# ag14774/OpenCL-Lattice-Boltzmann

Measured on AMD Instinct MI355X. Metric: MLUPS, higher is better.
Workload: dtype f32

## Files before the change

opencl-lattice-boltzmann_amd/csrc/core_interval.h:

```cpp
#pragma once

#if defined(__HIPCC__) || defined(__CUDACC__)
#define LBM_CORE_HD __host__ __device__ inline
#else
#define LBM_CORE_HD inline
#endif

namespace lbm {

struct CoreInterval {
  int kc0, kc1;
};

LBM_CORE_HD CoreInterval core_interval(int ys, int ye, int L, int ny, bool up, bool twinned, int accel_row, int accel_row_b,
                                       bool accel_next) {
  const int n = ye - ys, d = up ? 1 : -1;
  const int lead = twinned ? 0 : L - 1, sf = twinned ? 1 : 2;
  const int r0 = up ? ys - lead : ye - 1 + lead;
  const CoreInterval none = {0, 0};
  if (n <= 0 || L < 2) return none;
  int lo = lead + L - 1, hi = n + lead - 1;
  const int k_steady = sf * (L - 1) + 1;
  if (lo < k_steady) lo = k_steady;
  if (up) {
// ... 3 lines not shown
    if (lo < kmin) lo = kmin;
  } else {
    const int kmax = (r0 - 1) - 1;
    if (hi > kmax) hi = kmax;
    const int kmin = r0 - (ny - 2) - 1;
    if (lo < kmin) lo = kmin;
  }
  if (hi - lo + 1 < 2) return none;
  const int Lacc = accel_next ? L : L - 1;
  int c0[2], c1[2], nc = 0;
  const int arows[2] = {accel_row, accel_row_b};
  for (int i = 0; i < 2; i++) {
    const int A = arows[i];
    if (A < 0 || A >= ny || Lacc <= 0) continue;
    const int kA = (A - r0) * d;
    if (kA + Lacc - 1 < lo || kA > hi) continue;
    int j = nc++;
    if (j == 1 && kA < c0[0]) { c0[1] = c0[0]; c1[1] = c1[0]; j = 0; }
    c0[j] = kA;
    c1[j] = kA + Lacc - 1;
  }
  int best0 = 0, best1 = 0;
  int start = lo;
  for (int i = 0; i <= nc; i++) {
    const int end = i < nc ? c0[i] : hi + 1;
    if (end - start > best1 - best0) { best0 = start; best1 = end; }
    if (i < nc && c1[i] + 1 > start) start = c1[i] + 1;
  }
  if (best1 - best0 < 2) return none;
  const CoreInterval r = {best0, best1};
  return r;
}

}
```

opencl-lattice-boltzmann_amd/csrc/d2q9_kernels.h:

```cpp
#pragma once
#include <type_traits>

#include <hip/hip_runtime.h>
#include <stdint.h>

#include "core_interval.h"

namespace lbm {

constexpr int kBlock = 256;

struct StepArgs {
  const float *src;
  float *dst;
  const uint8_t *mask;
  const float *south_src[3];
  const float *north_src[3];
  float *partials;
  unsigned long long plane_stride;
  unsigned long long row_stride;
  int nx, rows;
  int y_begin, y_count;
  int y_split, y_begin2;
  int accel_row;
// ... 397 lines not shown
    }
  }
}

struct Step2Args {
  const float *src;
  float *dst;
  const uint8_t *mask;
  float *partials1;
  float *partials2;
  unsigned long long plane_stride, row_stride;
  int nx, ny;
  int strips, lanes_out;
  const int *chunk_start;
  int nchunks;
  int nbands, units_per_band;
  int skip_chunk;
  int accel_row;
  int accel_row_b;
  int accel_next;
  float omega, aw1, aw2;
  const int *edge_chunk_start;
  int edge_nchunks, edge_units, edge_skip;
  int edge_partial_off;
  const struct HaloPeer *peer;
  uint32_t seq, wait_seq;
  int peer_mode, peer_buf;
  const unsigned long long *clean_bits;
  int clean_words;
  const int *vmap;
  const int *vtab;
  int strips_edge;
  int core_loop;
};

struct UnitSel {
  const int *chunk_start;
  int bid, nbands, units_per_band, skip, partial_off;
  bool edge;
};
template <bool PUSH>
__device__ __forceinline__ UnitSel select_unit(const Step2Args &a, int edge_wgs) {
  UnitSel u{a.chunk_start, (int)blockIdx.x, a.nbands, a.units_per_band, a.skip_chunk, 0, false};
  if constexpr (PUSH) {
    if (u.bid < edge_wgs) {
      u.edge = true;
      u.chunk_start = a.edge_chunk_start;
      u.nbands = 1;
      u.units_per_band = edge_wgs;
      u.skip = a.edge_skip;
      u.partial_off = a.edge_partial_off;
    } else {
      u.bid -= edge_wgs;
    }
  }
  return u;
}

__device__ __forceinline__ void push_chunk(const Step2Args *la, int ys, int ye, int xcol, bool owner) {
  drain_stores();
  const HaloPeer *pp = uniform_ptr(la->peer);
  const int hi0 = __builtin_amdgcn_readfirstlane(pp->row_hi0);
  const int lo0 = __builtin_amdgcn_readfirstlane(pp->row_lo0);
  const int rows = __builtin_amdgcn_readfirstlane(pp->push_rows);
  const int buf = __builtin_amdgcn_readfirstlane(la->peer_buf) & 1;
  const int side = ys >= hi0 ? 1 : 0;
// ... 944 lines not shown
  float h0, h1, h2;
  uint32_t m;
};
template <bool NTL, bool HALO = true>
__device__ __forceinline__ void issue_pair_loads(const Step2Args &a, int r, int xcol, int xhalo_w, int xhalo_e, int lane, PairLoads &in) {
  const size_t ps = a.plane_stride, rs = a.row_stride;
  const int r_s = (r == 0) ? a.ny - 1 : r - 1;
  const int r_n = (r == a.ny - 1) ? 0 : r + 1;
  const float *Rc = a.src + (size_t)r * rs, *Rs = a.src + (size_t)r_s * rs, *Rn = a.src + (size_t)r_n * rs;
  unsigned xb = (unsigned)xcol * 4u;
  asm volatile("" : "+v"(xb));
  auto ld = [&](const float *p) {
    if (NTL) return __builtin_nontemporal_load(reinterpret_cast<const v2f *>(at_byte(p, xb)));
    return *reinterpret_cast<const v2f *>(at_byte(p, xb));
  };
  in.c[0] = ld(Rc); in.c[1] = ld(Rc + ps); in.c[3] = ld(Rc + 3 * ps);
  in.c[2] = ld(Rs + 2 * ps); in.c[5] = ld(Rs + 5 * ps); in.c[6] = ld(Rs + 6 * ps);
  in.c[4] = ld(Rn + 4 * ps); in.c[7] = ld(Rn + 7 * ps); in.c[8] = ld(Rn + 8 * ps);
  {
    unsigned mb = (unsigned)(xcol & ~3);
    asm volatile("" : "+v"(mb));
    in.m = *reinterpret_cast<const uint32_t *>(a.mask + (size_t)r * a.nx + mb);
  }
  in.h0 = in.h1 = in.h2 = 0.f;
  if (HALO && (lane == 0 || lane == 63)) {
    const bool lo = (lane == 0);
    in.h0 = lo ? Rc[1 * ps + xhalo_w] : Rc[3 * ps + xhalo_e];
    in.h1 = lo ? Rs[5 * ps + xhalo_w] : Rs[6 * ps + xhalo_e];
    in.h2 = lo ? Rn[8 * ps + xhalo_w] : Rn[7 * ps + xhalo_e];
  }
}

typedef __attribute__((address_space(1))) v2f global_v2f;
constexpr int kPairSlotFloats = 128;
constexpr int kPairWinFloats = 9 * kPairSlotFloats;
struct PairWindow { v2f mid[3], S0[3], S1[3]; };
struct __attribute__((packed, aligned(4))) f2u { float x, y; };
__device__ __forceinline__ v2f lds_pair(const float *p) { return *reinterpret_cast<const v2f *>(p); }
__device__ __forceinline__ v2f lds_pair_shifted(const float *p) {
  const f2u t = *reinterpret_cast<const f2u *>(p);
  v2f r = {t.x, t.y};
  return r;
}
__device__ __forceinline__ void lds_pair_put(float *p, v2f v) { *reinterpret_cast<v2f *>(p) = v; }

__device__ __forceinline__ void issue_pair_loads_at(const float *Rc, size_t ps, size_t rs, int xcol, PairLoads &in) {
  unsigned xb = (unsigned)xcol * 4u;
  asm volatile("" : "+v"(xb));
  auto ld = [&](const float *p) {
    unsigned long long pk = (unsigned long long)p;
    asm volatile("" : "+s"(pk));
    return *(const global_v2f *)(pk + xb);
  };
  const float *const Rs = Rc - rs, *const Rn = Rc + rs;
  in.c[0] = ld(Rc); in.c[1] = ld(Rc + ps); in.c[3] = ld(Rc + 3 * ps);
  in.c[2] = ld(Rs + 2 * ps); in.c[5] = ld(Rs + 5 * ps); in.c[6] = ld(Rs + 6 * ps);
  in.c[4] = ld(Rn + 4 * ps); in.c[7] = ld(Rn + 7 * ps); in.c[8] = ld(Rn + 8 * ps);
}

constexpr int deep_halo_lanes(int D) { return D / 2; }
constexpr bool deep_edge_loads(int D) { return 2 * deep_halo_lanes(D) < D; }
constexpr int deep_lds_windows(int D) { return D - 1 < 4 ? D - 1 : 4; }

__device__ __forceinline__ bool strip_rows_clean(const unsigned long long *bits, int words, int strip, int lo, int hi, int ny) {
  if (bits == nullptr || hi - lo >= ny) return false;
  const unsigned long long *w = bits + (size_t)strip * words;
  unsigned long long any = 0;
  auto range = [&](int r0, int r1) {
    for (int i = r0 >> 6; i <= (r1 - 1) >> 6; i++) {
      const int b0 = r0 - 64 * i > 0 ? r0 - 64 * i : 0, b1 = r1 - 64 * i < 64 ? r1 - 64 * i : 64;
      const unsigned long long upto = b1 == 64 ? ~0ull : ((1ull << b1) - 1ull);
      any |= w[i] & upto & ~((1ull << b0) - 1ull);
    }
  };
  int l0 = lo % ny;
  if (l0 < 0) l0 += ny;
  const int l1 = l0 + (hi - lo);
// ... 21 lines not shown
    const int r = word * 64 + b;
    if (r >= rows) break;
    const uint32_t m = *reinterpret_cast<const uint32_t *>(mask + (size_t)r * nx + (xcol & ~3)) >> ((xcol & 2) * 8);
    if (__builtin_amdgcn_ballot_w64((m & 0xffffu) != 0) != 0ull) out |= 1ull << b;
  }
  if (lane == 0) bits[(size_t)strip * words + word] = out;
}

template <int D, int WL, bool UP, bool NT, bool OBST_PATHS, bool TWIN = false, int LT = 0, bool FREE = false>
__device__ __forceinline__ void deep_sweep(const Step2Args &a, const int L_arg, float *lds, float *partials, int pstride, int ys, int ye,
                                           int xcol, int xhalo_w, int xhalo_e, int lane, bool owner, int unit,
                                           const bool twinned_in = false, float *lds_twin = nullptr) {
  static_assert(LT >= 0 && LT <= D, "steady depth");
  const int L = LT > 0 ? LT : L_arg;
  const bool twinned = TWIN && twinned_in;
  const size_t ps = a.plane_stride;
  auto wrap = [&](int r) { return r < 0 ? r + a.ny : (r >= a.ny ? r - a.ny : r); };
  const int n = ye - ys, d = UP ? 1 : -1;
  const int lead = twinned ? 0 : L - 1;
  const int sf = twinned ? 1 : 2;
  const int r0 = UP ? ys - lead : ye - 1 + lead;
  const int last = n + lead + (L - 1) - 1;
  float sum[D];
  constexpr int NR = (D - 1 - WL) > 0 ? (D - 1 - WL) : 1;
  PairWindow w[NR];
  uint32_t m_mid[D - 1];
#pragma unroll
  for (int l = 0; l < D; l++) sum[l] = 0.f;
#pragma unroll
  for (int l = 0; l < D - 1; l++) m_mid[l] = 0;
#pragma unroll
  for (int l = 0; l < NR; l++) {
#pragma unroll
    for (int i = 0; i < 3; i++) w[l].mid[i] = w[l].S0[i] = w[l].S1[i] = splat2(0.f);
  }
  float *const lw = lds + 2 + 2 * lane;
  uint32_t accbits = 0, ownbits = 0;
  const uint32_t accmask = a.accel_next ? 0xffffffffu : ~(1u << (L - 1));
  const uint32_t mask_shift = (xcol & 2) * 8;
  PairLoads in;
  issue_pair_loads<false, deep_edge_loads(D)>(a, wrap(r0), xcol, xhalo_w, xhalo_e, lane, in);
  float *const mailbox = lw + WL * kPairWinFloats;
  auto window_read = [&](int l, int par, int k, v2f (&q)[6]) __attribute__((always_inline)) {
    if ((l - 1) < WL) {
      const float *W = lw + (l - 1) * kPairWinFloats;
      const float *Wp = W + (3 + 3 * par) * kPairSlotFloats;
      q[0] = lds_pair(W); q[1] = lds_pair_shifted(W + kPairSlotFloats - 1); q[2] = lds_pair_shifted(W + 2 * kPairSlotFloats + 1);
      q[3] = lds_pair(Wp); q[4] = lds_pair_shifted(Wp + kPairSlotFloats - 1); q[5] = lds_pair_shifted(Wp + 2 * kPairSlotFloats + 1);
    } else {
      const PairWindow &R = w[(l - 1) < WL ? 0 : (l - 1 - WL)];
      q[0] = R.mid[0]; q[1] = pair_from_west(R.mid[1]); q[2] = pair_from_east(R.mid[2]);
      q[3] = R.S0[0]; q[4] = pair_from_west(R.S0[1]); q[5] = pair_from_east(R.S0[2]);
      if (TWIN && twinned && k == l) {
        q[3] = lds_pair(mailbox);
        q[4] = lds_pair_shifted(mailbox + kPairSlotFloats - 1);
        q[5] = lds_pair_shifted(mailbox + 2 * kPairSlotFloats + 1);
      }
    }
  };
  v2f out[9];
#pragma unroll
  for (int kk = 0; kk < 9; kk++) out[kk] = splat2(0.f);
  auto store_row_at = [&](float *const row) __attribute__((always_inline)) {
    if (owner) {
      unsigned xb = (unsigned)xcol * 4u;
      asm volatile("" : "+v"(xb));
#pragma unroll
      for (int kk = 0; kk < 9; kk++) {
        unsigned long long pk = (unsigned long long)(row + kk * ps);
        asm volatile("" : "+s"(pk));
        global_v2f *const q = (global_v2f *)(pk + xb);
        if (NT) __builtin_nontemporal_store(out[kk], q);
        else *q = out[kk];
      }
    }
  };
  auto store_row = [&](int kprev) __attribute__((always_inline)) { store_row_at(a.dst + (size_t)(r0 + (kprev - (L - 1)) * d) * a.row_stride); };
  constexpr bool HAS_CORE = LT > 0 && FREE && !deep_edge_loads(D);
  const float *core_src = a.src;
  float *core_dst = a.dst;
  const long long core_step = UP ? (long long)a.row_stride : -(long long)a.row_stride;
  auto iteration = [&](const int k, auto lt_tag, auto core_tag) __attribute__((always_inline)) {
    constexpr int LS = decltype(lt_tag)::value;
    constexpr bool STEADY = LS > 0;
    constexpr bool CORE = decltype(core_tag)::value;
    static_assert(!CORE || (STEADY && HAS_CORE), "the CORE form is a steady form of the free sweeps");
    const int LL = STEADY ? LS : L;
    const int par = k & 1;
    v2f top[9], pre[2][6];
    uint32_t m_top;
    if (!CORE) {
      const int row0 = wrap(r0 + k * d);
      accbits = ((accbits << 1) | ((row0 == a.accel_row || row0 == a.accel_row_b) ? 1u : 0u)) & accmask;
      ownbits = (ownbits << 1) | ((k >= lead && k <= n + lead - 1) ? 1u : 0u);
    }
    if (STEADY || k >= sf) window_read(1, par, STEADY ? -1 : k, pre[1]);
    {
      v2f g[9];
      g[0] = in.c[0]; g[2] = in.c[2]; g[4] = in.c[4];
      if (deep_edge_loads(D)) {
        g[1] = pair_from_west(in.c[1], in.h0); g[5] = pair_from_west(in.c[5], in.h1); g[8] = pair_from_west(in.c[8], in.h2);
        g[3] = pair_from_east(in.c[3], in.h0); g[6] = pair_from_east(in.c[6], in.h1); g[7] = pair_from_east(in.c[7], in.h2);
      } else {
        g[1] = pair_from_west(in.c[1]); g[5] = pair_from_west(in.c[5]); g[8] = pair_from_west(in.c[8]);
        g[3] = pair_from_east(in.c[3]); g[6] = pair_from_east(in.c[6]); g[7] = pair_from_east(in.c[7]);
      }
      m_top = FREE ? 0u : in.m >> mask_shift;
      v2f t;
      if (FREE || (OBST_PATHS && __builtin_amdgcn_ballot_w64((m_top & 0xffffu) != 0) == 0ull)) t = collide2<false>(g, m_top, a.omega, !CORE && (accbits & 1u) != 0, a.aw1, a.aw2, top);
      else t = collide2<true>(g, m_top, a.omega, (accbits & 1u) != 0, a.aw1, a.aw2, top);
      if ((CORE || (ownbits & 1u)) && owner) sum[0] += t.x + t.y;
      if (CORE) {
        store_row_at(core_dst);
        issue_pair_loads_at(core_src, ps, a.row_stride, xcol, in);
        core_dst += core_step;
        core_src += core_step;
      } else {
        if (STEADY || k - 1 >= sf * (LL - 1)) store_row(k - 1);
        issue_pair_loads<false, deep_edge_loads(D)>(a, wrap(r0 + (k < last ? k + 1 : k) * d), xcol, xhalo_w, xhalo_e, lane, in);
      }
    }
#pragma unroll
    for (int l = 1; l < D; l++) {
      if (STEADY && l >= LS) break;
      if (STEADY) __builtin_amdgcn_sched_barrier(0);
      const bool final = (l == D - 1) || (l == LL - 1);
      if (!STEADY && TWIN && (l - 1) >= WL && twinned && k == l) __syncthreads();
      v2f nxt[9];
      uint32_t m_nxt = 0;
      const bool active = STEADY || k >= sf * l;
      const bool in_lds = (l - 1) < WL;
      float *const W = lw + (l - 1) * kPairWinFloats;
      float *const Wp = W + (3 + 3 * par) * kPairSlotFloats;
      PairWindow &R = w[in_lds ? 0 : (l - 1 - WL)];
      if (active) {
        const v2f (&q)[6] = pre[l & 1];
        if (l + 1 < D && !final && (STEADY || k >= sf * (l + 1))) window_read(l + 1, par, STEADY ? -1 : k, pre[(l + 1) & 1]);
        v2f g[9];
        g[0] = q[0]; g[1] = q[1]; g[3] = q[2];
        if (UP) {
          g[2] = q[3]; g[5] = q[4]; g[6] = q[5];
          g[4] = top[4]; g[8] = pair_from_west(top[8]); g[7] = pair_from_east(top[7]);
        } else {
          g[4] = q[3]; g[8] = q[4]; g[7] = q[5];
          g[2] = top[2]; g[5] = pair_from_west(top[5]); g[6] = pair_from_east(top[6]);
        }
        m_nxt = FREE ? 0u : m_mid[l - 1];
        const bool acc = !CORE && ((accbits >> l) & 1u) != 0;
        v2f t;
        if (FREE || (OBST_PATHS && __builtin_amdgcn_ballot_w64((m_nxt & 0xffffu) != 0) == 0ull)) t = collide2<false>(g, m_nxt, a.omega, acc, a.aw1, a.aw2, nxt);
        else t = collide2<true>(g, m_nxt, a.omega, acc, a.aw1, a.aw2, nxt);
        if (!final) {
          if ((CORE || ((ownbits >> l) & 1u)) && owner) sum[l] += t.x + t.y;
        } else {
          if (owner) sum[l] += t.x + t.y;
#pragma unroll
          for (int kk = 0; kk < 9; kk++) out[kk] = nxt[kk];
        }
      }
      if (in_lds) {
        lds_pair_put(W, top[0]); lds_pair_put(W + kPairSlotFloats, top[1]); lds_pair_put(W + 2 * kPairSlotFloats, top[3]);
        lds_pair_put(Wp, UP ? top[2] : top[4]);
        lds_pair_put(Wp + kPairSlotFloats, UP ? top[5] : top[8]);
        lds_pair_put(Wp + 2 * kPairSlotFloats, UP ? top[6] : top[7]);
      } else {
        R.mid[0] = top[0]; R.mid[1] = top[1]; R.mid[2] = top[3];
#pragma unroll
        for (int i = 0; i < 3; i++) R.S0[i] = R.S1[i];
        R.S1[0] = UP ? top[2] : top[4]; R.S1[1] = UP ? top[5] : top[8]; R.S1[2] = UP ? top[6] : top[7];
      }
      if (!FREE) m_mid[l - 1] = m_top;
      if (!STEADY && TWIN && twinned && k == l - 1) {
        float *const Wt = lds_twin + 2 + 2 * lane + (in_lds ? (l - 1) * kPairWinFloats + (3 + 3 * (l & 1)) * kPairSlotFloats : WL * kPairWinFloats);
        lds_pair_put(Wt, UP ? top[4] : top[2]);
        lds_pair_put(Wt + kPairSlotFloats, UP ? top[8] : top[5]);
        lds_pair_put(Wt + 2 * kPairSlotFloats, UP ? top[7] : top[6]);
      }
      if (!active || final) break;
      if (l < D - 1) {
#pragma unroll
        for (int kk = 0; kk < 9; kk++) top[kk] = nxt[kk];
        m_top = m_nxt;
      }
    }
    if (!STEADY && TWIN && twinned && k <= L - 2) __syncthreads();
  };
  const int k_steady = sf * (L - 1) + 1;
  int k = 0;
  if (LT > 0) {
    for (; k < k_steady && k <= last; k++) iteration(k, std::integral_constant<int, 0>{}, std::false_type{});
    if constexpr (HAS_CORE) {
      CoreInterval ci = {0, 0};
      if (a.core_loop) ci = core_interval(ys, ye, L, a.ny, UP, twinned, a.accel_row, a.accel_row_b, a.accel_next != 0);
      const int kc0 = __builtin_amdgcn_readfirstlane(ci.kc0), kc1 = __builtin_amdgcn_readfirstlane(ci.kc1);
      bool core_ahead = kc1 > kc0;
      for (;;) {
        const int stop = core_ahead ? kc0 : last + 1;
        for (; k < stop; k++) iteration(k, std::integral_constant<int, LT>{}, std::false_type{});
        if (!core_ahead) break;
        core_ahead = false;
        core_src = a.src + (long long)(r0 + (kc0 + 1) * d) * (long long)a.row_stride;
        core_dst = a.dst + (long long)(r0 + (kc0 - L) * d) * (long long)a.row_stride;
        for (; k < kc1; k++) iteration(k, std::integral_constant<int, LT>{}, std::true_type{});
        ownbits = (1u << L) - 1u;
        accbits = 0;
      }
    } else {
      for (; k <= last; k++) iteration(k, std::integral_constant<int, LT>{}, std::false_type{});
    }
  } else {
    for (; k <= last; k++) iteration(k, std::integral_constant<int, 0>{}, std::false_type{});
  }
  store_row(last);
#pragma unroll
  for (int l = 0; l < D; l++) {
    if (l >= L) break;
    const float s = wave_sum(sum[l]);
    if (lane == 0) partials[(size_t)l * pstride + unit] = s;
  }
}

__device__ __forceinline__ void push_chunk_pairs(const Step2Args *la, int ys, int ye, int xcol, bool owner) {
  drain_stores();
  const HaloPeer *pp = uniform_ptr(la->peer);
  const int hi0 = __builtin_amdgcn_readfirstlane(pp->row_hi0);
  const int lo0 = __builtin_amdgcn_readfirstlane(pp->row_lo0);
  const int rows = __builtin_amdgcn_readfirstlane(pp->push_rows);
  const int buf = __builtin_amdgcn_readfirstlane(la->peer_buf) & 1;
  const int side = ys >= hi0 ? 1 : 0;
  const int base = side ? hi0 : lo0;
  if (ys < base || ye > base + rows) {
    if ((threadIdx.x & 63) == 0) atomicOr(pp->wait_err, 2u);
    return;
  }
  const size_t rs = la->row_stride, ps = la->plane_stride;
  const float *own = la->dst + xcol;
  float *peer = pp->push[side][buf] + xcol;
  if (owner) {
    for (int y = ys; y < ye; y++) {
      const float *src = own + (size_t)y * rs;
      float *dst = peer + (size_t)(y - base) * rs;
      v2f v[9];
#pragma unroll
      for (int k = 0; k < 9; k++) v[k] = *reinterpret_cast<const v2f *>(src + k * ps);
// ... 54 lines not shown
  if (qw < 0) qw += q2;
  const int xcol = qw * 2;
  const int xhalo_w = (xcol == 0) ? a.nx - 1 : xcol - 1;
  const int xhalo_e = (xcol + 2 >= a.nx) ? 0 : xcol + 2;
  const bool up = __builtin_amdgcn_readfirstlane((int)((chunk & 1) == 0)) != 0;
  bool clean = false;
  if constexpr (LT > 0 && OBST_PATHS) {
    int lo, hi;
    deep_sweep_rows(up, false, LT, ys, ye, &lo, &hi);
    clean = strip_rows_clean(a.clean_bits, a.clean_words, strip, lo, hi, a.ny);
  }
  if (clean) {
    if constexpr (LT > 0 && OBST_PATHS) {
      if (up) deep_sweep<D, WL, true, NT, OBST_PATHS, false, LT, true>(a, nlev, lds, partials, pstride, ys, ye, xcol, xhalo_w, xhalo_e, lane, owner, unit);
      else deep_sweep<D, WL, false, NT, OBST_PATHS, false, LT, true>(a, nlev, lds, partials, pstride, ys, ye, xcol, xhalo_w, xhalo_e, lane, owner, unit);
    }
  } else if (up) {
    deep_sweep<D, WL, true, NT, OBST_PATHS, false, LT>(a, nlev, lds, partials, pstride, ys, ye, xcol, xhalo_w, xhalo_e, lane, owner, unit);
  } else {
    deep_sweep<D, WL, false, NT, OBST_PATHS, false, LT>(a, nlev, lds, partials, pstride, ys, ye, xcol, xhalo_w, xhalo_e, lane, owner, unit);
  }
  if constexpr (PUSH) {
    const Step2Args *la = late_args<Step2Args>();
    if (do_push) {
      push_chunk_pairs(la, ys, ye, xcol, owner);
      publish_wave_when_last(la->peer, (unsigned)la->edge_units, la->seq);
    }
  }
}

template <int D, bool NT, bool OBST_PATHS = false, int LT = 0, bool PUSH = false>
__global__ __launch_bounds__(128, 2) void d2q9_deep_twin(const Step2Args a, float *partials, int pstride, int nlev) {
  constexpr int WL = deep_lds_windows(D), HL = deep_halo_lanes(D);
  constexpr int kWaveFloats = WL * kPairWinFloats + (D - 1 > WL ? 3 * kPairSlotFloats : 0) + 4;
  constexpr bool EDGE_PAIRS = PUSH && D <= 5;
  __shared__ float lds[2 * kWaveFloats];
  const int lane = threadIdx.x & 63;
  const int wv = __builtin_amdgcn_readfirstlane((int)(threadIdx.x >> 6));
  const UnitSel us = select_unit<PUSH>(a, a.edge_units / 2);
  const bool do_push = PUSH && us.edge && (a.peer_mode & 1);
  if constexpr (PUSH) {
    if (us.edge && (a.peer_mode & 2)) {
      const Step2Args *la = late_args<Step2Args>();
      const HaloPeer *pp = la->peer;
      if (lane < 2) spin_on_flag(pp->wait_flags + lane, la->wait_seq, pp->wait_err, pp->wait_ticks);
    }
  }
  const int band = us.bid % us.nbands, slot = us.bid / us.nbands;
  if (slot >= us.units_per_band) return;
  const int punit = band * us.units_per_band + slot;
  const bool edge_wg = PUSH && us.edge;
  const int sdiv = edge_wg ? a.strips_edge : a.strips;
  const int pair = punit / sdiv;
  int strip = punit - pair * sdiv;
  const int chunk = edge_wg ? (EDGE_PAIRS ? 4 * pair + wv : 2 * wv) : 2 * pair + wv;
  const int unit = ((edge_wg && EDGE_PAIRS) ? 2 * pair + wv : chunk) * sdiv + strip + us.partial_off;
  int ys, ye, pys, pye;
  if (a.vmap != nullptr && !edge_wg) {
    const int *e = a.vtab + 2 * ((size_t)a.vmap[2 * strip + 1] * a.nchunks + chunk), *pe = e + (wv ? -2 : 2);
    strip = a.vmap[2 * strip];
    ys = e[0]; ye = e[1];
    pys = pe[0]; pye = pe[1];
  } else {
    ys = us.chunk_start[chunk]; ye = us.chunk_start[chunk + 1];
    pys = us.chunk_start[chunk ^ 1]; pye = us.chunk_start[(chunk ^ 1) + 1];
  }
  const bool empty = ys >= ye || (!(PUSH && us.edge) && chunk == us.skip);
// ... 517 lines not shown
```

opencl-lattice-boltzmann_amd/csrc/lbm_hip.cpp:

```cpp
#include "../../include/lbm.h"
#include "d2q9_kernels.h"
#include "deep_instances.h"
#include "chunk_schedule.h"
#include "halo_exchange.h"
#include "lbm_error.h"

#include <dlfcn.h>
#include <rccl/rccl.h>
#include <unistd.h>

#include <algorithm>
#include <cmath>
#include <cstdarg>
#include <cstdio>
#include <cstdlib>
#include <cstring>
#include <string>
#include <vector>

namespace {

thread_local std::string g_err;

int fail(int code, const char *fmt, ...) {
// ... 210 lines not shown
  int halo_depth = 3;
  int rank = 0;
  int cur = 0;
  int steps_done = 0;
  int ring_fill = 0;
  int ring = kRingMax;
  int transport_eff = TRANSPORT_COPY;
  uint32_t halo_seq = 0;
  int halo_sync = 0;
  unsigned long long halo_timeout_ms = kHaloWaitMsDefault;
  int compact = -1;
  int push_release = -1;
  int stale_exchange = 0;
  bool failed = false;
  std::vector<hipEvent_t> prof_ev;
  int prof_sets = -1;
  int variant = 0;
  int grid_blocks = 0;
  int nt_stores = -1;
  int nt_loads = -1;
  int fuse = -1;
  int tile_shape = -1;
  int windows = -1;
  int load_bufs = 0;
  int sched_waves = 0;
  int pair = -1;
  int twin_steps = 0;
  int edge_aware = -1;
  int steady = -1;
  int obst_paths = -1;
  int balance = -1;
  int free_sweeps = -1;
  int core_loop = -1;
  int multistep = -1;
  int resident = -1;
  int chunk_rows = 0;
  int chunk_min = 0;
  int pair_taper = -1;
  bool vec4 = true;
  double *av_host = nullptr;
};

namespace {

using namespace lbm;

int div_up(long a, long b) { return (int)((a + b - 1) / b); }

int set_dev(const Slab &s) {
  HIP_TRY(hipSetDevice(s.dev));
  return LBM_OK;
}

template <typename T>
int dev_alloc(T **p, size_t count) {
  HIP_TRY(hipMalloc(reinterpret_cast<void **>(p), count * sizeof(T)));
  return LBM_OK;
}

int step_blocks(const lbm_ctx *c, int work_rows) {
  const int vec = c->vec4 ? 4 : 1;
  const long threads = (long)(c->p.nx / vec) * work_rows;
  int nb = div_up(threads, kBlock);
  if (c->grid_blocks > 0) nb = std::min(nb, c->grid_blocks);
  return std::max(1, nb);
}
// ... 620 lines not shown
  a.omega = c->p.omega;
  a.aw1 = c->p.density * c->p.accel / 9.0f;
  a.aw2 = c->p.density * c->p.accel / 36.0f;
  for (int k = 0; k < 3; k++) {
    static const int sp[3] = {2, 5, 6}, np[3] = {4, 7, 8};
    a.south_src[k] = s.cells[src] + sp[k] * s.plane_stride + (size_t)(s.ext_rows - 1) * s.row_stride;
    a.north_src[k] = s.cells[src] + np[k] * s.plane_stride;
  }
  return a;
}

Step2Args base_args2(const lbm_ctx *c, const Slab &s, int src, bool accel_next, const FuseGeom &g) {
  Step2Args a{};
  a.src = s.cells[src];
  a.dst = s.cells[src ^ 1];
  a.mask = s.mask;
  a.plane_stride = s.plane_stride;
  a.row_stride = s.row_stride;
  a.nx = c->p.nx;
  a.ny = s.ext_rows;
  a.strips = s.strips;
  a.lanes_out = s.lanes_out;
  a.chunk_start = g.chunk_start;
  a.vmap = g.vmap;
  a.vtab = g.vtab;
  a.nchunks = g.nchunks;
  a.nbands = g.nbands;
  a.units_per_band = g.units_per_band;
  a.skip_chunk = -1;
  a.accel_row = s.accel_ext;
  a.accel_row_b = s.accel_ext_b;
  a.accel_next = accel_next ? 1 : 0;
  a.core_loop = c->core_loop != 0 ? 1 : 0;
  a.omega = c->p.omega;
  a.aw1 = c->p.density * c->p.accel / 9.0f;
  a.aw2 = c->p.density * c->p.accel / 36.0f;
  return a;
}

void launch_step3(const Step2Args &a0, float *partials3, int units, hipStream_t st, bool paired = false) {
  if (paired) {
    Step2Args a = a0;
    a.units_per_band = a0.units_per_band / 2;
    hipLaunchKernelGGL((d2q9_step3p<true, 0>), dim3(units / 2), dim3(128), 0, st, a, partials3);
    return;
  }
  hipLaunchKernelGGL((d2q9_step3<true, 0, true, 1>), dim3(units), dim3(64), 0, st, a0, partials3);
}

void launch_step4(const Step2Args &a0, float *partials3, float *partials4, int units, hipStream_t st, bool paired = false) {
  if (paired) {
    Step2Args a = a0;
    a.units_per_band = a0.units_per_band / 2;
    hipLaunchKernelGGL((d2q9_step4p<true, 0>), dim3(units / 2), dim3(128), 0, st, a, partials3, partials4);
    return;
  }
  hipLaunchKernelGGL((d2q9_step4<true, 0>), dim3(units), dim3(64), 0, st, a0, partials3, partials4);
}

using DeepKernel = void (*)(const Step2Args, float *, int, int);
enum DeepFamily {
  DEEP_LONE,
  DEEP_LONE_PUSH,
  DEEP_TWIN8,
  DEEP_TWIN8_PUSH,
  DEEP_TWIN5,
// ... 1464 lines not shown
  }
  if (!strcmp(key, "edge_aware")) {
    if (value < -1 || value > 1) return fail(LBM_ERR_ARG, "edge_aware must be -1 (auto), 0 or 1");
    if (int rc = sync_all(c)) return rc;
    c->edge_aware = (int)value;
    return rebuild_geometry(c);
  }
  if (!strcmp(key, "steady")) {
    if (value < -1 || value > 1) return fail(LBM_ERR_ARG, "steady must be -1 (auto), 0 or 1");
    c->steady = (int)value;
    return LBM_OK;
  }
  if (!strcmp(key, "obst_paths")) {
    if (value < -1 || value > 1) return fail(LBM_ERR_ARG, "obst_paths must be -1 (auto), 0 or 1");
    c->obst_paths = (int)value;
    return LBM_OK;
  }
  if (!strcmp(key, "balance")) {
    if (value < -1 || value > 1) return fail(LBM_ERR_ARG, "balance must be -1 (auto), 0 or 1");
    if (int rc = sync_all(c)) return rc;
    c->balance = (int)value;
    return rebuild_geometry(c);
  }
  if (!strcmp(key, "free_sweeps")) {
    if (value < -1 || value > 1) return fail(LBM_ERR_ARG, "free_sweeps must be -1 (auto), 0 or 1");
    c->free_sweeps = (int)value;
    return LBM_OK;
  }
  if (!strcmp(key, "core_loop")) {
    if (value < -1 || value > 1) return fail(LBM_ERR_ARG, "core_loop must be -1 (auto), 0 or 1");
    c->core_loop = (int)value;
    return LBM_OK;
  }
  if (!strcmp(key, "tile_shape")) {
    if (value < -1 || value > 2) return fail(LBM_ERR_ARG, "tile_shape must be -1..2");
    if (int rc = sync_all(c)) return rc;
    c->tile_shape = (int)value;
    return rebuild_geometry(c);
  }
  if (!strcmp(key, "pair")) {
    if (int rc = sync_all(c)) return rc;
    c->pair = (int)value;
    return rebuild_geometry(c);
  }
  if (!strcmp(key, "windows") || !strcmp(key, "load_bufs") || !strcmp(key, "sched_waves")) {
    if (value < -1 || value > 2) return fail(LBM_ERR_ARG, "%s out of range", key);
    if (key[0] == 'w' && value == 0) return fail(LBM_ERR_ARG, "windows 0 (register windows of d2q9_step3) was removed: -1 or 1");
    if (key[0] == 'l' && value == 2) return fail(LBM_ERR_ARG, "load_bufs 2 (two row-sets of loads in flight in d2q9_step3) was removed: 0 or 1");
    if (int rc = sync_all(c)) return rc;
    (key[0] == 'w' ? c->windows : (key[0] == 'l' ? c->load_bufs : c->sched_waves)) = (int)value;
    return rebuild_geometry(c);
  }
  if (!strcmp(key, "transport")) {
    if (!c->halo_mode) return fail(LBM_ERR_STATE, "a context without halo rows has no transport");
    if (int rc = sync_all(c)) return rc;
    if (value == TRANSPORT_RCCL) {
      for (const Slab &s : c->slabs)
        if (!s.comm) return fail(LBM_ERR_STATE, "no RCCL communicator: create the context with a comm_id (or default transport 1)");
    } else if (value == TRANSPORT_PEER) {
      for (const Slab &s : c->slabs)
        if (!s.south.connected || !s.north.connected) return fail(LBM_ERR_STATE, "peers are not connected (lbm_connect_peers)");
    } else {
      return fail(LBM_ERR_ARG, "transport must be 1 (RCCL send/recv) or 3 (peer stores)");
    }
    c->transport_eff = (int)value;
    return rebuild_geometry(c);
// ... 78 lines not shown
    c->pair_taper = (int)value;
    return rebuild_geometry(c);
  }
  return fail(LBM_ERR_ARG, "unknown option '%s'", key);
}

int lbm_get_option(const lbm_ctx *c, const char *key, long *value) {
  if (!c || !key || !value) return fail(LBM_ERR_ARG, "NULL argument");
  const LaunchPlan p = resolve_plan(c);
  const Slab *s0 = c->slabs.empty() ? nullptr : &c->slabs[0];
  if (!strcmp(key, "variant")) *value = effective_mode(c) + 1;
  else if (!strcmp(key, "grid_blocks")) *value = s0 ? s0->nb_main : 0;
  else if (!strcmp(key, "nt_stores")) *value = nt_effective(c);
  else if (!strcmp(key, "fuse")) *value = p.fuse_lvl >= 3 ? p.fuse_lvl : (p.fuse_lvl ? 1 : 0);
  else if (!strcmp(key, "multistep")) *value = p.kind == KIND_MULTI ? p.cap : 0;
  else if (!strcmp(key, "resident")) *value = p.kind == KIND_RESIDENT ? s0->res_bh : 0;
  else if (!strcmp(key, "chunk_rows")) *value = c->chunk_rows;
  else if (!strcmp(key, "pair_taper")) *value = pair_taper(c);
  else if (!strcmp(key, "windows")) *value = windows_in_lds(c);
  else if (!strcmp(key, "pair")) *value = p.pairs;
  else if (!strcmp(key, "load_bufs")) *value = step3_load_bufs(c);
  else if (!strcmp(key, "launch_steps")) *value = p.cap;
  else if (!strcmp(key, "fuse_units"))
    *value = !s0 ? 0 : (p.twin ? s0->f6_main.units : set_geom(p, *s0, p.window_kind).main->units) + set_geom(p, *s0, p.window_kind).edge->units;
  else if (!strcmp(key, "transport")) *value = c->transport_eff;
  else if (!strcmp(key, "steady")) *value = c->steady != 0;
  else if (!strcmp(key, "balance")) {
    const int vstrips = s0 && p.fuse_lvl >= kDeepMin ? set_geom(p, *s0, KIND_DEEP).main->vstrips : 0;
    *value = vstrips > 0 ? vstrips - s0->strips2 : 0;
  }
  else if (!strcmp(key, "free_sweeps"))
    *value = s0 && p.fuse_lvl >= kDeepMin && clean_bits_for(c, *s0, *set_geom(p, *s0, KIND_DEEP).main) != nullptr;
  else if (!strcmp(key, "core_loop")) *value = c->core_loop != 0;
  else if (!strcmp(key, "halo_sync")) *value = c->halo_sync;
  else if (!strcmp(key, "halo_timeout_ms")) *value = (long)c->halo_timeout_ms;
  else if (!strcmp(key, "push_release")) *value = c->slabs.empty() ? 0 : push_release_effective(c, c->slabs[0]);
  else if (!strcmp(key, "debug_stale_exchange")) *value = c->stale_exchange;
  else if (!strcmp(key, "compact")) *value = p.compact();
  else if (!strcmp(key, "halo_depth")) *value = c->halo_mode ? c->halo_depth : 0;
  else if (!strcmp(key, "nslabs")) *value = c->nslabs_global;
  else if (!strcmp(key, "cus")) *value = s0 ? s0->cus : 0;
  else return fail(LBM_ERR_ARG, "unknown option '%s'", key);
  return LBM_OK;
}

int lbm_valu_rate(int launches, double *tera_lane_instr_per_s) {
  if (!tera_lane_instr_per_s || launches < 1) return fail(LBM_ERR_ARG, "bad argument");
  const int nb = 256 * 8, iters = 4096;
  float *out = nullptr;
  HIP_TRY(hipMalloc((void **)&out, (size_t)nb * kBlock * sizeof(float)));
  hipEvent_t t0, t1;
  hipEventCreate(&t0);
  hipEventCreate(&t1);
  hipLaunchKernelGGL(lbm::valu_spin, dim3(nb), dim3(kBlock), 0, 0, out, iters, 0.5f);
  hipEventRecord(t0, 0);
  for (int i = 0; i < launches; i++) hipLaunchKernelGGL(lbm::valu_spin, dim3(nb), dim3(kBlock), 0, 0, out, iters, 0.5f);
  hipEventRecord(t1, 0);
  const hipError_t e = hipEventSynchronize(t1);
  float ms = 0.f;
  hipEventElapsedTime(&ms, t0, t1);
  hipEventDestroy(t0);
  hipEventDestroy(t1);
  hipFree(out);
  if (e != hipSuccess || ms <= 0.f) return fail(LBM_ERR_HIP, "valu_spin: %s", hipGetErrorString(e));
  *tera_lane_instr_per_s = (double)nb * kBlock * (double)iters * 32.0 * launches / (ms * 1e-3) / 1e12;
  return LBM_OK;
// ... 72 lines not shown
```

Measured before the change: 484,000.

## Unroll core sweep loop by row pairs with compile-time parity and reorganize LDS windows

Adds a core_unroll option (on by default) that splits the core interval into an even-aligned run of row pairs, each iterated with a compile-time row parity. Register windows then index their trailing slots statically instead of shifting S0/S1 every row. The LDS window layout is regrouped into per-row blocks of west/east/place slots, read through a single 32-bit LDS base with address-space-3 pointers so the loads can use immediate offsets. This is meant to remove register moves and address arithmetic from the hot loop, at the cost of more code size and possible register pressure.

```diff
diff --git a/opencl-lattice-boltzmann_amd/csrc/core_interval.h b/opencl-lattice-boltzmann_amd/csrc/core_interval.h
--- a/opencl-lattice-boltzmann_amd/csrc/core_interval.h
+++ b/opencl-lattice-boltzmann_amd/csrc/core_interval.h
@@ -59,4 +59,16 @@
   return r;
 }
 
+struct CorePairs {
+  int ke0, ke1;
+};
+
+LBM_CORE_HD CorePairs core_pairs(int kc0, int kc1) {
+  CorePairs p = {kc0, kc0};
+  if (kc1 <= kc0) return p;
+  p.ke0 = kc0 + (kc0 & 1);
+  p.ke1 = p.ke0 + ((kc1 - p.ke0) & ~1);
+  return p;
 }
+
+}
diff --git a/opencl-lattice-boltzmann_amd/csrc/d2q9_kernels.h b/opencl-lattice-boltzmann_amd/csrc/d2q9_kernels.h
--- a/opencl-lattice-boltzmann_amd/csrc/d2q9_kernels.h
+++ b/opencl-lattice-boltzmann_amd/csrc/d2q9_kernels.h
@@ -453,6 +453,7 @@
   const int *vtab;
   int strips_edge;
   int core_loop;
+  int core_unroll;
 };
 
 struct UnitSel {
@@ -1463,17 +1464,29 @@
 }
 
 typedef __attribute__((address_space(1))) v2f global_v2f;
+typedef __attribute__((address_space(3))) float lds_float;
+typedef float v2f_a4 __attribute__((ext_vector_type(2), aligned(4)));
 constexpr int kPairSlotFloats = 128;
-constexpr int kPairWinFloats = 9 * kPairSlotFloats;
-struct PairWindow { v2f mid[3], S0[3], S1[3]; };
-struct __attribute__((packed, aligned(4))) f2u { float x, y; };
-__device__ __forceinline__ v2f lds_pair(const float *p) { return *reinterpret_cast<const v2f *>(p); }
-__device__ __forceinline__ v2f lds_pair_shifted(const float *p) {
-  const f2u t = *reinterpret_cast<const f2u *>(p);
-  v2f r = {t.x, t.y};
-  return r;
-}
+constexpr int kPairRowFloats = 3 * kPairSlotFloats;
+constexpr int kPairWinFloats = 3 * kPairRowFloats;
+constexpr int kPairSlotWest = 0, kPairSlotEast = 1, kPairSlotPlace = 2;
+constexpr int pair_row_mid() { return 0; }
+constexpr int pair_row_trail(int par) { return (1 + par) * kPairRowFloats; }
+struct PairWindow { v2f mid[3], S[2][3]; };
 __device__ __forceinline__ void lds_pair_put(float *p, v2f v) { *reinterpret_cast<v2f *>(p) = v; }
+__device__ __forceinline__ void lds_row_get(unsigned lane_base, int row, v2f &place, v2f &west, v2f &east) {
+  unsigned b = lane_base + (unsigned)(row - 1) * 4u;
+  asm volatile("" : "+v"(b));
+  const lds_float *const B = (const lds_float *)(size_t)b;
+  west = *reinterpret_cast<const __attribute__((address_space(3))) v2f_a4 *>(B + kPairSlotWest * kPairSlotFloats);
+  east = *reinterpret_cast<const __attribute__((address_space(3))) v2f_a4 *>(B + kPairSlotEast * kPairSlotFloats + 2);
+  place = *reinterpret_cast<const __attribute__((address_space(3))) v2f *>(B + kPairSlotPlace * kPairSlotFloats + 1);
+}
+__device__ __forceinline__ void lds_row_put(float *row, v2f place, v2f west, v2f east) {
+  lds_pair_put(row + kPairSlotPlace * kPairSlotFloats, place);
+  lds_pair_put(row + kPairSlotWest * kPairSlotFloats, west);
+  lds_pair_put(row + kPairSlotEast * kPairSlotFloats, east);
+}
 
 __device__ __forceinline__ void issue_pair_loads_at(const float *Rc, size_t ps, size_t rs, int xcol, PairLoads &in) {
   unsigned xb = (unsigned)xcol * 4u;
@@ -1561,7 +1574,7 @@
 #pragma unroll
   for (int l = 0; l < NR; l++) {
 #pragma unroll
-    for (int i = 0; i < 3; i++) w[l].mid[i] = w[l].S0[i] = w[l].S1[i] = splat2(0.f);
+    for (int i = 0; i < 3; i++) w[l].mid[i] = w[l].S[0][i] = w[l].S[1][i] = splat2(0.f);
   }
   float *const lw = lds + 2 + 2 * lane;
   uint32_t accbits = 0, ownbits = 0;
@@ -1569,22 +1582,17 @@
   const uint32_t mask_shift = (xcol & 2) * 8;
   PairLoads in;
   issue_pair_loads<false, deep_edge_loads(D)>(a, wrap(r0), xcol, xhalo_w, xhalo_e, lane, in);
-  float *const mailbox = lw + WL * kPairWinFloats;
-  auto window_read = [&](int l, int par, int k, v2f (&q)[6]) __attribute__((always_inline)) {
+  unsigned lw_row = (unsigned)(size_t)(lds_float *)lw;
+  auto window_read = [&](int l, int par, int spar, int k, v2f (&q)[6]) __attribute__((always_inline)) {
     if ((l - 1) < WL) {
-      const float *W = lw + (l - 1) * kPairWinFloats;
-      const float *Wp = W + (3 + 3 * par) * kPairSlotFloats;
-      q[0] = lds_pair(W); q[1] = lds_pair_shifted(W + kPairSlotFloats - 1); q[2] = lds_pair_shifted(W + 2 * kPairSlotFloats + 1);
-      q[3] = lds_pair(Wp); q[4] = lds_pair_shifted(Wp + kPairSlotFloats - 1); q[5] = lds_pair_shifted(Wp + 2 * kPairSlotFloats + 1);
+      const int W = (l - 1) * kPairWinFloats;
+      lds_row_get(lw_row, W + pair_row_mid(), q[0], q[1], q[2]);
+      lds_row_get(lw_row, W + pair_row_trail(par), q[3], q[4], q[5]);
     } else {
       const PairWindow &R = w[(l - 1) < WL ? 0 : (l - 1 - WL)];
       q[0] = R.mid[0]; q[1] = pair_from_west(R.mid[1]); q[2] = pair_from_east(R.mid[2]);
-      q[3] = R.S0[0]; q[4] = pair_from_west(R.S0[1]); q[5] = pair_from_east(R.S0[2]);
-      if (TWIN && twinned && k == l) {
-        q[3] = lds_pair(mailbox);
-        q[4] = lds_pair_shifted(mailbox + kPairSlotFloats - 1);
-        q[5] = lds_pair_shifted(mailbox + 2 * kPairSlotFloats + 1);
-      }
+      q[3] = R.S[spar][0]; q[4] = pair_from_west(R.S[spar][1]); q[5] = pair_from_east(R.S[spar][2]);
+      if (TWIN && twinned && k == l) lds_row_get(lw_row, WL * kPairWinFloats, q[3], q[4], q[5]);
     }
   };
   v2f out[9];
@@ -1609,13 +1617,17 @@
   const float *core_src = a.src;
   float *core_dst = a.dst;
   const long long core_step = UP ? (long long)a.row_stride : -(long long)a.row_stride;
-  auto iteration = [&](const int k, auto lt_tag, auto core_tag) __attribute__((always_inline)) {
+  auto iteration = [&](const int k, auto lt_tag, auto core_tag, auto par_tag) __attribute__((always_inline)) {
     constexpr int LS = decltype(lt_tag)::value;
     constexpr bool STEADY = LS > 0;
     constexpr bool CORE = decltype(core_tag)::value;
+    constexpr int PT = decltype(par_tag)::value;
     static_assert(!CORE || (STEADY && HAS_CORE), "the CORE form is a steady form of the free sweeps");
+    static_assert(PT == -1 || ((PT == 0 || PT == 1) && CORE), "a compile-time row parity is the CORE form's");
     const int LL = STEADY ? LS : L;
-    const int par = k & 1;
+    const int par = PT >= 0 ? PT : (k & 1);
+    asm volatile("" : "+v"(lw_row));
+    constexpr int spar = PT >= 0 ? PT : 0;
     v2f top[9], pre[2][6];
     uint32_t m_top;
     if (!CORE) {
@@ -1623,7 +1635,7 @@
       accbits = ((accbits << 1) | ((row0 == a.accel_row || row0 == a.accel_row_b) ? 1u : 0u)) & accmask;
       ownbits = (ownbits << 1) | ((k >= lead && k <= n + lead - 1) ? 1u : 0u);
     }
-    if (STEADY || k >= sf) window_read(1, par, STEADY ? -1 : k, pre[1]);
+    if (STEADY || k >= sf) window_read(1, par, spar, STEADY ? -1 : k, pre[1]);
     {
       v2f g[9];
       g[0] = in.c[0]; g[2] = in.c[2]; g[4] = in.c[4];
@@ -1660,11 +1672,10 @@
       const bool active = STEADY || k >= sf * l;
       const bool in_lds = (l - 1) < WL;
       float *const W = lw + (l - 1) * kPairWinFloats;
-      float *const Wp = W + (3 + 3 * par) * kPairSlotFloats;
       PairWindow &R = w[in_lds ? 0 : (l - 1 - WL)];
       if (active) {
         const v2f (&q)[6] = pre[l & 1];
-        if (l + 1 < D && !final && (STEADY || k >= sf * (l + 1))) window_read(l + 1, par, STEADY ? -1 : k, pre[(l + 1) & 1]);
+        if (l + 1 < D && !final && (STEADY || k >= sf * (l + 1))) window_read(l + 1, par, spar, STEADY ? -1 : k, pre[(l + 1) & 1]);
         v2f g[9];
         g[0] = q[0]; g[1] = q[1]; g[3] = q[2];
         if (UP) {
@@ -1688,22 +1699,21 @@
         }
       }
       if (in_lds) {
-        lds_pair_put(W, top[0]); lds_pair_put(W + kPairSlotFloats, top[1]); lds_pair_put(W + 2 * kPairSlotFloats, top[3]);
-        lds_pair_put(Wp, UP ? top[2] : top[4]);
-        lds_pair_put(Wp + kPairSlotFloats, UP ? top[5] : top[8]);
-        lds_pair_put(Wp + 2 * kPairSlotFloats, UP ? top[6] : top[7]);
+        lds_row_put(W + pair_row_mid(), top[0], top[1], top[3]);
+        lds_row_put(W + pair_row_trail(par), UP ? top[2] : top[4], UP ? top[5] : top[8], UP ? top[6] : top[7]);
       } else {
         R.mid[0] = top[0]; R.mid[1] = top[1]; R.mid[2] = top[3];
-#pragma unroll
-        for (int i = 0; i < 3; i++) R.S0[i] = R.S1[i];
-        R.S1[0] = UP ? top[2] : top[4]; R.S1[1] = UP ? top[5] : top[8]; R.S1[2] = UP ? top[6] : top[7];
+        if (PT < 0) {
+#pragma unroll
+          for (int i = 0; i < 3; i++) R.S[0][i] = R.S[1][i];
+        }
+        constexpr int snew = PT >= 0 ? PT : 1;
+        R.S[snew][0] = UP ? top[2] : top[4]; R.S[snew][1] = UP ? top[5] : top[8]; R.S[snew][2] = UP ? top[6] : top[7];
       }
       if (!FREE) m_mid[l - 1] = m_top;
       if (!STEADY && TWIN && twinned && k == l - 1) {
-        float *const Wt = lds_twin + 2 + 2 * lane + (in_lds ? (l - 1) * kPairWinFloats + (3 + 3 * (l & 1)) * kPairSlotFloats : WL * kPairWinFloats);
-        lds_pair_put(Wt, UP ? top[4] : top[2]);
-        lds_pair_put(Wt + kPairSlotFloats, UP ? top[8] : top[5]);
-        lds_pair_put(Wt + 2 * kPairSlotFloats, UP ? top[7] : top[6]);
+        float *const Wt = lds_twin + 2 + 2 * lane + (in_lds ? (l - 1) * kPairWinFloats + pair_row_trail(l & 1) : WL * kPairWinFloats);
+        lds_row_put(Wt, UP ? top[4] : top[2], UP ? top[8] : top[5], UP ? top[7] : top[6]);
       }
       if (!active || final) break;
       if (l < D - 1) {
@@ -1715,9 +1725,10 @@
     if (!STEADY && TWIN && twinned && k <= L - 2) __syncthreads();
   };
   const int k_steady = sf * (L - 1) + 1;
+  constexpr std::integral_constant<int, -1> kParRun{};
   int k = 0;
   if (LT > 0) {
-    for (; k < k_steady && k <= last; k++) iteration(k, std::integral_constant<int, 0>{}, std::false_type{});
+    for (; k < k_steady && k <= last; k++) iteration(k, std::integral_constant<int, 0>{}, std::false_type{}, kParRun);
     if constexpr (HAS_CORE) {
       CoreInterval ci = {0, 0};
       if (a.core_loop) ci = core_interval(ys, ye, L, a.ny, UP, twinned, a.accel_row, a.accel_row_b, a.accel_next != 0);
@@ -1725,20 +1736,33 @@
       bool core_ahead = kc1 > kc0;
       for (;;) {
         const int stop = core_ahead ? kc0 : last + 1;
-        for (; k < stop; k++) iteration(k, std::integral_constant<int, LT>{}, std::false_type{});
+        for (; k < stop; k++) iteration(k, std::integral_constant<int, LT>{}, std::false_type{}, kParRun);
         if (!core_ahead) break;
         core_ahead = false;
         core_src = a.src + (long long)(r0 + (kc0 + 1) * d) * (long long)a.row_stride;
         core_dst = a.dst + (long long)(r0 + (kc0 - L) * d) * (long long)a.row_stride;
-        for (; k < kc1; k++) iteration(k, std::integral_constant<int, LT>{}, std::true_type{});
+        CorePairs cp = {kc1, kc1};
+        if (a.core_unroll) cp = core_pairs(kc0, kc1);
+        const int ke0 = __builtin_amdgcn_readfirstlane(cp.ke0), ke1 = __builtin_amdgcn_readfirstlane(cp.ke1);
+        for (int part = 0; part < 2; part++) {
+          const int single_stop = part == 0 ? ke0 : kc1;
+          for (; k < single_stop; k++) iteration(k, std::integral_constant<int, LT>{}, std::true_type{}, kParRun);
+          if (part == 0) {
+            for (; k < ke1; k += 2) {
+              iteration(k, std::integral_constant<int, LT>{}, std::true_type{}, std::integral_constant<int, 0>{});
+              __builtin_amdgcn_sched_barrier(0);
+              iteration(k + 1, std::integral_constant<int, LT>{}, std::true_type{}, std::integral_constant<int, 1>{});
+            }
+          }
+        }
         ownbits = (1u << L) - 1u;
         accbits = 0;
       }
     } else {
-      for (; k <= last; k++) iteration(k, std::integral_constant<int, LT>{}, std::false_type{});
+      for (; k <= last; k++) iteration(k, std::integral_constant<int, LT>{}, std::false_type{}, kParRun);
     }
   } else {
-    for (; k <= last; k++) iteration(k, std::integral_constant<int, 0>{}, std::false_type{});
+    for (; k <= last; k++) iteration(k, std::integral_constant<int, 0>{}, std::false_type{}, kParRun);
   }
   store_row(last);
 #pragma unroll
@@ -1859,7 +1883,7 @@
 template <int D, bool NT, bool OBST_PATHS = false, int LT = 0, bool PUSH = false>
 __global__ __launch_bounds__(128, 2) void d2q9_deep_twin(const Step2Args a, float *partials, int pstride, int nlev) {
   constexpr int WL = deep_lds_windows(D), HL = deep_halo_lanes(D);
-  constexpr int kWaveFloats = WL * kPairWinFloats + (D - 1 > WL ? 3 * kPairSlotFloats : 0) + 4;
+  constexpr int kWaveFloats = WL * kPairWinFloats + (D - 1 > WL ? kPairRowFloats : 0) + 4;
   constexpr bool EDGE_PAIRS = PUSH && D <= 5;
   __shared__ float lds[2 * kWaveFloats];
   const int lane = threadIdx.x & 63;
diff --git a/opencl-lattice-boltzmann_amd/csrc/lbm_hip.cpp b/opencl-lattice-boltzmann_amd/csrc/lbm_hip.cpp
--- a/opencl-lattice-boltzmann_amd/csrc/lbm_hip.cpp
+++ b/opencl-lattice-boltzmann_amd/csrc/lbm_hip.cpp
@@ -266,6 +266,7 @@
   int balance = -1;
   int free_sweeps = -1;
   int core_loop = -1;
+  int core_unroll = -1;
   int multistep = -1;
   int resident = -1;
   int chunk_rows = 0;
@@ -952,6 +953,7 @@
   a.accel_row_b = s.accel_ext_b;
   a.accel_next = accel_next ? 1 : 0;
   a.core_loop = c->core_loop != 0 ? 1 : 0;
+  a.core_unroll = c->core_unroll != 0 ? 1 : 0;
   a.omega = c->p.omega;
   a.aw1 = c->p.density * c->p.accel / 9.0f;
   a.aw2 = c->p.density * c->p.accel / 36.0f;
@@ -2482,6 +2484,11 @@
     c->core_loop = (int)value;
     return LBM_OK;
   }
+  if (!strcmp(key, "core_unroll")) {
+    if (value < -1 || value > 1) return fail(LBM_ERR_ARG, "core_unroll must be -1 (auto), 0 or 1");
+    c->core_unroll = (int)value;
+    return LBM_OK;
+  }
   if (!strcmp(key, "tile_shape")) {
     if (value < -1 || value > 2) return fail(LBM_ERR_ARG, "tile_shape must be -1..2");
     if (int rc = sync_all(c)) return rc;
@@ -2626,6 +2633,7 @@
   else if (!strcmp(key, "free_sweeps"))
     *value = s0 && p.fuse_lvl >= kDeepMin && clean_bits_for(c, *s0, *set_geom(p, *s0, KIND_DEEP).main) != nullptr;
   else if (!strcmp(key, "core_loop")) *value = c->core_loop != 0;
+  else if (!strcmp(key, "core_unroll")) *value = c->core_unroll != 0;
   else if (!strcmp(key, "halo_sync")) *value = c->halo_sync;
   else if (!strcmp(key, "halo_timeout_ms")) *value = (long)c->halo_timeout_ms;
   else if (!strcmp(key, "push_release")) *value = c->slabs.empty() ? 0 : push_release_effective(c, c->slabs[0]);
```

After: 486,400 (median of 6 runs). No clear change (+0.5%).
